# jihun1998/AO

Hardware: AMD Instinct MI355X
Metric: points/sec fwd+bwd PTv2m2 S3DIS (higher is better)
Workload: dtype fp32

## Files before the change

ao_amd/csrc/gva_fwd_tile.hip:

```cpp
#include <algorithm>
#include <cstdlib>

#include "gva_common.h"

namespace gva {

typedef float ft_v4f __attribute__((ext_vector_type(4)));
__device__ __forceinline__ ft_v4f ft_mfma(float a, float b, ft_v4f c) { return __builtin_amdgcn_mfma_f32_16x16x4f32(a, b, c, 0, 0, 0); }
template <int CTRL>
__device__ __forceinline__ float ft_dpp(float v) {
    return __int_as_float(__builtin_amdgcn_update_dpp(0, __float_as_int(v), CTRL, 0xF, 0xF, true));
}
__device__ __forceinline__ float ft_row16_sum(float v) {
    v += ft_dpp<0xB1>(v);
    v += ft_dpp<0x4E>(v);
    v += ft_dpp<0x141>(v);
    v += ft_dpp<0x140>(v);
    return v;
}
__device__ __forceinline__ float ft_row16_max(float v) {
    v = fmaxf(v, ft_dpp<0xB1>(v));
    v = fmaxf(v, ft_dpp<0x4E>(v));
    v = fmaxf(v, ft_dpp<0x141>(v));
    v = fmaxf(v, ft_dpp<0x140>(v));
    return v;
}
__device__ __forceinline__ void ft_wave_sync() {
    asm volatile("s_waitcnt lgkmcnt(0)" ::: "memory");
    __builtin_amdgcn_wave_barrier();
}

__host__ __device__ constexpr int ft_ww_pitch(int G) {
    int p = G;
    while (p % 16 != 4) ++p;
    return p;
}
__host__ __device__ constexpr int ft_point_pitch(int GB, int GP) {
    int p = GB * GP;
    while (p % 64 != 4) p += 4;
    return p;
}

template <int G, int C, int GB>
struct FwdTileCfg {
    static constexpr int GTF = (G + 15) / 16, G16 = GTF * 16, GPW = ft_ww_pitch(G), QB = GB / 4, NGW = GB / 4, OB = 8 * GB,
                         NCH = C / 16, GP = 20, PP = ft_point_pitch(GB, GP), OP = OB + 4, WT = 16 * 17;
    static_assert(GB % 4 == 0 && GB <= 16 && G % GB == 0 && C == 8 * G && GPW >= G16, "group blocks of 4 q groups");
    static constexpr size_t lds_floats = 4 * (size_t)C + 4 * 256 + 16 * GPW + 16 + 2 * G16 + 16 * WT + 256 + 2 * 16 * PP + 16 * OP;
};

template <int G, int C, int GB, bool WRITE_A, bool DROP>
__global__ __launch_bounds__(256, 2) void attention_fwd_tile_kernel(
    int n, const float *__restrict__ W1, const float *__restrict__ sc, const float *__restrict__ sh, const float *__restrict__ Ww2,
    const float *__restrict__ bw2, const float *__restrict__ v, const float *__restrict__ a, const float *__restrict__ b,
    const float *__restrict__ coord, const int *__restrict__ idx, const float *__restrict__ Wp2, const float *__restrict__ bp2,
    float *__restrict__ w, float *__restrict__ sw, float *__restrict__ out, float *__restrict__ stats, float *__restrict__ a_out,
    PtvDrop drop) {
    using K = FwdTileCfg<G, C, GB>;
    constexpr int GTF = K::GTF, G16 = K::G16, GPW = K::GPW, QB = K::QB, NGW = K::NGW, OB = K::OB, NCH = K::NCH, GP = K::GP, PP = K::PP,
                  OP = K::OP, WT = K::WT;
    extern __shared__ float4 lds4[];
    float4 *sAB = lds4;
    float4 *sPos = sAB + C;
    float *sWw = (float *)(sPos + 256);
    float *sBw = sWw + 16 * GPW;
    float *sSc = sBw + 16;
    float *sSh = sSc + G16;
    float *sWt = sSh + G16;
    float *sSw = sWt + 16 * WT;
    float *sA = sSw + 256;
    float *sOut = sA + 2 * 16 * PP;

    const int tid = threadIdx.x, lane = tid & 63, wid = tid >> 6, l15 = lane & 15, q = lane >> 4;
    const int tile = blockIdx.x, g0 = blockIdx.y * GB, o0 = 8 * g0;
    const long long last = (long long)n - 1;

    long long pts[4];
    int srcv[4];
    float u[4][GTF][4];
#pragma unroll
    for (int i = 0; i < 4; ++i) {
        const long long pt = (long long)tile * 16 + 4 * wid + i;
        pts[i] = pt < n ? pt : last;
        srcv[i] = idx[pts[i] * 16 + l15];
        const float *row = W1 + (pts[i] * 16 + l15) * G;
#pragma unroll
        for (int t = 0; t < GTF; ++t) {
            const int j0 = 16 * t + 4 * q;
            const float4 uu = *(const float4 *)(row + (j0 < G ? j0 : 0));
            u[i][t][0] = j0 < G ? uu.x : 0.f; u[i][t][1] = j0 < G ? uu.y : 0.f;
            u[i][t][2] = j0 < G ? uu.z : 0.f; u[i][t][3] = j0 < G ? uu.w : 0.f;
        }
    }
    for (int ch = tid; ch < C; ch += 256) sAB[ch] = make_float4(a[3 * ch], a[3 * ch + 1], a[3 * ch + 2], b[ch]);
    for (int e = tid; e < 16 * GPW; e += 256) {
        const int row = e / GPW, j = e - row * GPW;
        sWw[e] = (row < GB && j < G) ? Ww2[(g0 + row) * G + j] : 0.f;
    }
    if (tid < 16) sBw[tid] = tid < GB ? bw2[g0 + tid] : 0.f;
    for (int j = tid; j < G16; j += 256) { sSc[j] = j < G ? sc[j] : 0.f; sSh[j] = j < G ? sh[j] : 0.f; }
    float cx[4], cy[4], cz[4];
#pragma unroll
    for (int i = 0; i < 4; ++i) {
        const long long ss = srcv[i] >= 0 ? srcv[i] : 0;
        cx[i] = coord[3 * ss] - coord[3 * pts[i]];
        cy[i] = coord[3 * ss + 1] - coord[3 * pts[i] + 1];
        cz[i] = coord[3 * ss + 2] - coord[3 * pts[i] + 2];
    }
    const int of = lane & 31, par = lane >> 5;
    const bool fa = of < OB / 4;
    auto request_rows = [&](int i, float4 (&rows)[8]) {
#pragma unroll
        for (int j = 0; j < 8; ++j) {
            const int s0 = __builtin_amdgcn_readlane(srcv[i], 2 * j), s1 = __builtin_amdgcn_readlane(srcv[i], 2 * j + 1);
            const int src = par ? s1 : s0;
            const float *vp = (fa && src >= 0) ? v + (long long)src * C + o0 + 4 * of : ptv2_zero_pad;
            rows[j] = *(const float4 *)vp;
        }
    };
    auto reduce_rows = [&](int i, const float4 (&rows)[8]) {
        const int p = 4 * wid + i, gl = fa ? of >> 1 : 0;
        float wg[8];
#pragma unroll
        for (int j = 0; j < 8; ++j) wg[j] = sWt[p * WT + gl * 17 + 2 * j + par];
        float4 acc = make_float4(0.f, 0.f, 0.f, 0.f);
#pragma unroll
        for (int j = 0; j < 8; ++j) {
            acc.x = __builtin_fmaf(wg[j], rows[j].x, acc.x); acc.y = __builtin_fmaf(wg[j], rows[j].y, acc.y);
            acc.z = __builtin_fmaf(wg[j], rows[j].z, acc.z); acc.w = __builtin_fmaf(wg[j], rows[j].w, acc.w);
        }
        acc.x += __shfl_xor(acc.x, 32, WAVE); acc.y += __shfl_xor(acc.y, 32, WAVE);
        acc.z += __shfl_xor(acc.z, 32, WAVE); acc.w += __shfl_xor(acc.w, 32, WAVE);
        if (par == 0 && fa) *(float4 *)(sOut + p * OP + 4 * of) = acc;
    };
    float4 vv0[8], vv1[8];
#ifndef FT_SKIP_OUTV
    request_rows(0, vv0);
    request_rows(1, vv1);
#endif
    __syncthreads();

    ft_v4f z[4];
#pragma unroll
    for (int i = 0; i < 4; ++i) z[i] = (ft_v4f){0.f, 0.f, 0.f, 0.f};
#pragma unroll
    for (int t = 0; t < GTF; ++t) {
        const float4 s4 = *(const float4 *)(sSc + 16 * t + 4 * q), h4 = *(const float4 *)(sSh + 16 * t + 4 * q);
        const float4 w4 = *(const float4 *)(sWw + l15 * GPW + 16 * t + 4 * q);
#pragma unroll
        for (int i = 0; i < 4; ++i) z[i] = ft_mfma(w4.x, fmaxf(__builtin_fmaf(s4.x, u[i][t][0], h4.x), 0.f), z[i]);
#pragma unroll
        for (int i = 0; i < 4; ++i) z[i] = ft_mfma(w4.y, fmaxf(__builtin_fmaf(s4.y, u[i][t][1], h4.y), 0.f), z[i]);
#pragma unroll
        for (int i = 0; i < 4; ++i) z[i] = ft_mfma(w4.z, fmaxf(__builtin_fmaf(s4.z, u[i][t][2], h4.z), 0.f), z[i]);
#pragma unroll
        for (int i = 0; i < 4; ++i) z[i] = ft_mfma(w4.w, fmaxf(__builtin_fmaf(s4.w, u[i][t][3], h4.w), 0.f), z[i]);
    }
    const float4 b4 = *(const float4 *)(sBw + 4 * q);
    const float bb[4] = {b4.x, b4.y, b4.z, b4.w};
#pragma unroll
    for (int i = 0; i < 4; ++i) {
        const int p = 4 * wid + i;
        const bool valid = srcv[i] >= 0;
        float wv[4], so[4];
#pragma unroll
        for (int r = 0; r < 4; ++r) {
            const float zz = z[i][r] + bb[r];
            const float mx = ft_row16_max(zz);
            const float e = expf(zz - mx);
            const float den = ft_row16_sum(e);
            wv[r] = (valid && q < QB) ? e / den : 0.f;
            if (DROP) wv[r] *= ptv2_drop_factor(drop, ((unsigned long long)pts[i] * 16 + l15) * G + (g0 + 4 * q + r));
            so[r] = ft_row16_sum(wv[r]);
            sWt[p * WT + (4 * q + r) * 17 + l15] = wv[r];
        }
        if (q < QB) {
            *(float4 *)(w + (pts[i] * 16 + l15) * G + g0 + 4 * q) = make_float4(wv[0], wv[1], wv[2], wv[3]);
            if (l15 == 0) {
                *(float4 *)(sw + pts[i] * G + g0 + 4 * q) = make_float4(so[0], so[1], so[2], so[3]);
                *(float4 *)(sSw + p * 16 + 4 * q) = make_float4(so[0], so[1], so[2], so[3]);
            }
        }
        sPos[p * 16 + l15] = valid ? make_float4(cx[i], cy[i], cz[i], 0.f) : make_float4(0.f, 0.f, 0.f, 0.f);
    }
    ft_wave_sync();

#ifndef FT_SKIP_OUTV
    reduce_rows(0, vv0);
    reduce_rows(1, vv1);
    request_rows(2, vv0);
    request_rows(3, vv1);
#endif

    float wA[4][4];
    float3 pq[4][4];
#pragma unroll
    for (int i = 0; i < 4; ++i)
#pragma unroll
        for (int st = 0; st < 4; ++st) {
            wA[i][st] = sWt[(4 * wid + i) * WT + l15 * 17 + 4 * st + q];
            const float4 t = sPos[(4 * wid + i) * 16 + 4 * st + q];
            pq[i][st] = make_float3(t.x, t.y, t.z);
        }
    const float *wp2row[NGW];
    float4 wpn[NGW];
    ft_v4f acc[NGW];
#pragma unroll
    for (int gi = 0; gi < NGW; ++gi) {
        const int g = wid + 4 * gi;
        wp2row[gi] = Wp2 + (size_t)(o0 + 8 * g + (l15 & 7)) * C + 4 * q;
        wpn[gi] = *(const float4 *)wp2row[gi];
        acc[gi] = (ft_v4f){0.f, 0.f, 0.f, 0.f};
    }
#ifdef FT_SKIP_CHUNKS
    __syncthreads();
#else
#pragma unroll 2
    for (int ck = 0; ck < NCH; ++ck) {
        float *buf = sA + (ck & 1) * 16 * PP;
        float4 wpc[NGW];
        const int cn = ck + 1 < NCH ? ck + 1 : ck;
#pragma unroll
        for (int gi = 0; gi < NGW; ++gi) { wpc[gi] = wpn[gi]; wpn[gi] = *(const float4 *)(wp2row[gi] + 16 * cn); }
        const float4 ab = sAB[16 * ck + l15];
        ft_v4f d[4];
#pragma unroll
        for (int i = 0; i < 4; ++i) d[i] = (ft_v4f){0.f, 0.f, 0.f, 0.f};
#pragma unroll
        for (int st = 0; st < 4; ++st)
#pragma unroll
            for (int i = 0; i < 4; ++i)
                d[i] = ft_mfma(wA[i][st], pe_act(ab.x, ab.y, ab.z, ab.w, pq[i][st].x, pq[i][st].y, pq[i][st].z), d[i]);
        if (q < QB) {
#pragma unroll
            for (int i = 0; i < 4; ++i)
#pragma unroll
                for (int r = 0; r < 4; ++r) buf[(4 * wid + i) * PP + (4 * q + r) * GP + l15] = d[i][r];
            if constexpr (WRITE_A) {
#pragma unroll
                for (int i = 0; i < 4; ++i)
#pragma unroll
                    for (int r = 0; r < 4; ++r) a_out[(pts[i] * G + g0 + 4 * q + r) * C + 16 * ck + l15] = d[i][r];
            }
        }
        __syncthreads();
#pragma unroll
        for (int gi = 0; gi < NGW; ++gi) {
            const float4 bx = *(const float4 *)(buf + l15 * PP + (wid + 4 * gi) * GP + 4 * q);
            acc[gi] = ft_mfma(wpc[gi].x, bx.x, acc[gi]);
            acc[gi] = ft_mfma(wpc[gi].y, bx.y, acc[gi]);
            acc[gi] = ft_mfma(wpc[gi].z, bx.z, acc[gi]);
            acc[gi] = ft_mfma(wpc[gi].w, bx.w, acc[gi]);
        }
    }
#endif

#ifndef FT_SKIP_OUTV
    reduce_rows(2, vv0);
    reduce_rows(3, vv1);
#endif
    __syncthreads();
    const long long ptl = (long long)tile * 16 + l15;
    const bool rv = ptl < n;
    const int cnt = (int)std::min<long long>(16, (long long)n - (long long)tile * 16);
    const float inv = 1.0f / (float)cnt;
#pragma unroll
    for (int gi = 0; gi < NGW; ++gi) {
        const int g = wid + 4 * gi;
        if (q < 2) {
            const int ol = 8 * g + 4 * q;
            const float4 ov = *(const float4 *)(sOut + l15 * OP + ol);
            const float s = sSw[l15 * 16 + g];
            const float4 bb = *(const float4 *)(bp2 + o0 + ol);
            float4 val;
            val.x = ov.x + acc[gi][0] + bb.x * s; val.y = ov.y + acc[gi][1] + bb.y * s;
            val.z = ov.z + acc[gi][2] + bb.z * s; val.w = ov.w + acc[gi][3] + bb.w * s;
            if (rv) *(float4 *)(out + ptl * C + o0 + ol) = val;
            if (stats) {
                const float s0 = ft_row16_sum(rv ? val.x : 0.f), s1 = ft_row16_sum(rv ? val.y : 0.f);
                const float s2 = ft_row16_sum(rv ? val.z : 0.f), s3 = ft_row16_sum(rv ? val.w : 0.f);
                const float d0 = rv ? val.x - s0 * inv : 0.f, d1 = rv ? val.y - s1 * inv : 0.f;
                const float d2 = rv ? val.z - s2 * inv : 0.f, d3 = rv ? val.w - s3 * inv : 0.f;
                const float m0 = ft_row16_sum(d0 * d0), m1 = ft_row16_sum(d1 * d1), m2 = ft_row16_sum(d2 * d2), m3 = ft_row16_sum(d3 * d3);
                if (l15 == 0) {
                    float *rec = stats + (size_t)tile * 2 * C + o0 + ol;
                    *(float4 *)rec = make_float4(s0, s1, s2, s3);
                    *(float4 *)(rec + C) = make_float4(m0, m1, m2, m3);
                }
            }
        }
    }
}

template <int G, int C, int GB>
static int launch_fwd_tile(int n, const float *W1, const float *sc, const float *sh, const float *Ww2, const float *bw2, const float *v,
                           const float *a, const float *b, const float *coord, const int *idx, const float *Wp2, const float *bp2,
                           float *w, float *sw, float *out, float *stats, float *a_out, PtvDrop drop, hipStream_t st) {
    using K = FwdTileCfg<G, C, GB>;
    const size_t lds = sizeof(float) * K::lds_floats;
    const bool dropping = drop.thresh != 0;
    auto kern = a_out ? (dropping ? attention_fwd_tile_kernel<G, C, GB, true, true> : attention_fwd_tile_kernel<G, C, GB, true, false>)
                      : (dropping ? attention_fwd_tile_kernel<G, C, GB, false, true> : attention_fwd_tile_kernel<G, C, GB, false, false>);
    static bool configured[2][2] = {{false, false}, {false, false}};
    if (!configured[a_out != nullptr][dropping]) {
        if (hipFuncSetAttribute((const void *)kern, hipFuncAttributeMaxDynamicSharedMemorySize, (int)lds) != hipSuccess) return PTV2_ERR_LAUNCH;
        configured[a_out != nullptr][dropping] = true;
    }
    hipLaunchKernelGGL(kern, dim3((n + 15) / 16, G / GB), dim3(256), lds, st, n, W1, sc, sh, Ww2, bw2, v, a, b, coord, idx, Wp2, bp2, w,
                       sw, out, stats, a_out, drop);
    return PTV2_OK;
}

}

int gva_fwd_tile_supported(int k, int c, int g) {
    return k == 16 && ((g == 12 && c == 96) || (g == 24 && c == 192) || (g == 48 && c == 384) || (g == 64 && c == 512));
}
int gva_fwd_tile_stat_rows() { return 16; }

int gva_fwd_tile_launch(int n, int k, int c, int g, const float *W1, const float *sc, const float *sh, const float *Ww2,
                        const float *bw2, const float *v, const float *a, const float *b, const float *coord, const int *idx,
                        const float *Wp2, const float *bp2, float *w, float *sw, float *out, float *stats, float *a_out, void *stream) {
    using namespace gva;
    if (!gva_fwd_tile_supported(k, c, g) || n < 1) return PTV2_ERR_ARG;
    hipStream_t st = (hipStream_t)stream;
    PtvScopedTimer t(KID_FWD_TILE + (g == 12 ? 0 : g == 24 ? 1 : g == 48 ? 2 : 3), st,
                     4.0 * ((double)n * k * (2 * g + 1) + (double)n * (3 + 2 * c + g)));
    int rc;
    const PtvDrop drop = ptv2_attn_drop_current();
#define ARGS n, W1, sc, sh, Ww2, bw2, v, a, b, coord, idx, Wp2, bp2, w, sw, out, stats, a_out, drop, st
    if (g == 12) rc = launch_fwd_tile<12, 96, 12>(ARGS);
    else if (g == 24) rc = launch_fwd_tile<24, 192, 12>(ARGS);
    else if (g == 48) rc = launch_fwd_tile<48, 384, 12>(ARGS);
    else rc = launch_fwd_tile<64, 512, 16>(ARGS);
#undef ARGS
    if (rc != PTV2_OK) return rc;
    PTV2_CHECK_LAUNCH();
    return PTV2_OK;
}

extern "C" int gva_attention_forward_hip_launcher(int n, int k, int c, int g, const float *W1, const float *sc, const float *sh,
                                                  const float *Ww2, const float *bw2, const float *v, const float *a,
                                                  const float *b, const float *coord, const int *idx, const float *Wp2,
                                                  const float *bp2, float *w, float *sw, float *out, float *A, void *stream) {
    if (!W1 || !sc || !sh || !Ww2 || !bw2 || !v || !a || !b || !coord || !idx || !Wp2 || !bp2 || !w || !sw || !out) return PTV2_ERR_ARG;
    if (n == 0) return PTV2_OK;
    return gva_fwd_tile_launch(n, k, c, g, W1, sc, sh, Ww2, bw2, v, a, b, coord, idx, Wp2, bp2, w, sw, out, nullptr, A, stream);
}
```

Baseline: 12.81 million.

## Choose forward tile group-block geometry per size to balance CU wave rounds

Turns the forward attention tile kernel into a 1D-grid dispatcher that can run two group-block sizes in one launch. The first tiles use the wide block, the tail uses GB=4. A host-side planner picks the block sizes and split point from the CU count, using a simple cost model (rounds × (fixed + GB)) to cut tail-wave imbalance. An environment override is added. The cost is more template instantiations, a max-LDS allocation across both configs, and divide/mod index math per block.

```diff
diff --git a/ao_amd/csrc/gva_fwd_tile.hip b/ao_amd/csrc/gva_fwd_tile.hip
--- a/ao_amd/csrc/gva_fwd_tile.hip
+++ b/ao_amd/csrc/gva_fwd_tile.hip
@@ -1,5 +1,6 @@
 #include <algorithm>
 #include <cstdlib>
+#include <cstring>
 
 #include "gva_common.h"
 
@@ -50,12 +51,12 @@
 };
 
 template <int G, int C, int GB, bool WRITE_A, bool DROP>
-__global__ __launch_bounds__(256, 2) void attention_fwd_tile_kernel(
+__device__ __forceinline__ void attention_fwd_tile_body(
     int n, const float *__restrict__ W1, const float *__restrict__ sc, const float *__restrict__ sh, const float *__restrict__ Ww2,
     const float *__restrict__ bw2, const float *__restrict__ v, const float *__restrict__ a, const float *__restrict__ b,
     const float *__restrict__ coord, const int *__restrict__ idx, const float *__restrict__ Wp2, const float *__restrict__ bp2,
     float *__restrict__ w, float *__restrict__ sw, float *__restrict__ out, float *__restrict__ stats, float *__restrict__ a_out,
-    PtvDrop drop) {
+    PtvDrop drop, const int tile, const int g0) {
     using K = FwdTileCfg<G, C, GB>;
     constexpr int GTF = K::GTF, G16 = K::G16, GPW = K::GPW, QB = K::QB, NGW = K::NGW, OB = K::OB, NCH = K::NCH, GP = K::GP, PP = K::PP,
                   OP = K::OP, WT = K::WT;
@@ -72,7 +73,7 @@
     float *sOut = sA + 2 * 16 * PP;
 
     const int tid = threadIdx.x, lane = tid & 63, wid = tid >> 6, l15 = lane & 15, q = lane >> 4;
-    const int tile = blockIdx.x, g0 = blockIdx.y * GB, o0 = 8 * g0;
+    const int o0 = 8 * g0;
     const long long last = (long long)n - 1;
 
     long long pts[4];
@@ -292,23 +293,83 @@
     }
 }
 
-template <int G, int C, int GB>
-static int launch_fwd_tile(int n, const float *W1, const float *sc, const float *sh, const float *Ww2, const float *bw2, const float *v,
-                           const float *a, const float *b, const float *coord, const int *idx, const float *Wp2, const float *bp2,
-                           float *w, float *sw, float *out, float *stats, float *a_out, PtvDrop drop, hipStream_t st) {
-    using K = FwdTileCfg<G, C, GB>;
-    const size_t lds = sizeof(float) * K::lds_floats;
+template <int G, int C, int GB1, int GB2, bool WRITE_A, bool DROP>
+__global__ __launch_bounds__(256, 2) void attention_fwd_tile_kernel(
+    int n, int nt1, int nwg1, const float *__restrict__ W1, const float *__restrict__ sc, const float *__restrict__ sh,
+    const float *__restrict__ Ww2, const float *__restrict__ bw2, const float *__restrict__ v, const float *__restrict__ a,
+    const float *__restrict__ b, const float *__restrict__ coord, const int *__restrict__ idx, const float *__restrict__ Wp2,
+    const float *__restrict__ bp2, float *__restrict__ w, float *__restrict__ sw, float *__restrict__ out, float *__restrict__ stats,
+    float *__restrict__ a_out, PtvDrop drop) {
+    const int bid = blockIdx.x;
+    if (GB1 == GB2 || bid < nwg1) {
+        attention_fwd_tile_body<G, C, GB1, WRITE_A, DROP>(n, W1, sc, sh, Ww2, bw2, v, a, b, coord, idx, Wp2, bp2, w, sw, out, stats,
+                                                          a_out, drop, bid % nt1, bid / nt1 * GB1);
+    } else if constexpr (GB1 != GB2) {
+        const int nt2 = (n + 15) / 16 - nt1, r = bid - nwg1;
+        attention_fwd_tile_body<G, C, GB2, WRITE_A, DROP>(n, W1, sc, sh, Ww2, bw2, v, a, b, coord, idx, Wp2, bp2, w, sw, out, stats,
+                                                          a_out, drop, nt1 + r % nt2, r / nt2 * GB2);
+    }
+}
+
+template <int G, int C, int GB1, int GB2>
+static int launch_fwd_tile(int n, int nt1, const float *W1, const float *sc, const float *sh, const float *Ww2, const float *bw2,
+                           const float *v, const float *a, const float *b, const float *coord, const int *idx, const float *Wp2,
+                           const float *bp2, float *w, float *sw, float *out, float *stats, float *a_out, PtvDrop drop, hipStream_t st) {
+    const size_t lds = sizeof(float) * std::max(FwdTileCfg<G, C, GB1>::lds_floats, FwdTileCfg<G, C, GB2>::lds_floats);
     const bool dropping = drop.thresh != 0;
-    auto kern = a_out ? (dropping ? attention_fwd_tile_kernel<G, C, GB, true, true> : attention_fwd_tile_kernel<G, C, GB, true, false>)
-                      : (dropping ? attention_fwd_tile_kernel<G, C, GB, false, true> : attention_fwd_tile_kernel<G, C, GB, false, false>);
+    auto kern = a_out ? (dropping ? attention_fwd_tile_kernel<G, C, GB1, GB2, true, true> : attention_fwd_tile_kernel<G, C, GB1, GB2, true, false>)
+                      : (dropping ? attention_fwd_tile_kernel<G, C, GB1, GB2, false, true> : attention_fwd_tile_kernel<G, C, GB1, GB2, false, false>);
     static bool configured[2][2] = {{false, false}, {false, false}};
     if (!configured[a_out != nullptr][dropping]) {
         if (hipFuncSetAttribute((const void *)kern, hipFuncAttributeMaxDynamicSharedMemorySize, (int)lds) != hipSuccess) return PTV2_ERR_LAUNCH;
         configured[a_out != nullptr][dropping] = true;
     }
-    hipLaunchKernelGGL(kern, dim3((n + 15) / 16, G / GB), dim3(256), lds, st, n, W1, sc, sh, Ww2, bw2, v, a, b, coord, idx, Wp2, bp2, w,
-                       sw, out, stats, a_out, drop);
+    const int nt = (n + 15) / 16;
+    if (GB1 == GB2) nt1 = nt;
+    const int nwg1 = nt1 * (G / GB1), nwg = nwg1 + (nt - nt1) * (G / GB2);
+    hipLaunchKernelGGL(kern, dim3(nwg), dim3(256), lds, st, n, nt1, nwg1, W1, sc, sh, Ww2, bw2, v, a, b, coord, idx, Wp2, bp2, w, sw,
+                       out, stats, a_out, drop);
     return PTV2_OK;
+}
+
+struct FtPlan { int gb1, gb2, nt1; };
+constexpr int FT_FIXED = 16;
+
+static int ft_cus() {
+    static const int cus = [] {
+        int dev = 0, c = 0;
+        if (hipGetDevice(&dev) != hipSuccess || hipDeviceGetAttribute(&c, hipDeviceAttributeMultiprocessorCount, dev) != hipSuccess || c < 1) c = 256;
+        return c;
+    }();
+    return cus;
+}
+static const char *ft_geom_env() {
+    static const char *e = [] { const char *v = getenv("AO_AMD_FT_GEOM"); return (v && v[0] && strcmp(v, "auto") != 0) ? v : (const char *)nullptr; }();
+    return e;
+}
+static FtPlan ft_plan(int n, int G, int gbdef, const int *cands, int ncand) {
+    const int nt = (n + 15) / 16, cus = ft_cus();
+    auto rounds = [cus](long long wg) { return (long long)((wg + cus - 1) / cus); };
+    auto whole = [&](int gb) { return (long long)nt * (G / gb) / cus * cus / (G / gb); };
+    if (const char *e = ft_geom_env()) {
+        const int gb = e[0] == '0' ? gbdef : atoi(e);
+        bool ok = false;
+        for (int i = 0; i < ncand; ++i) ok |= cands[i] == gb;
+        if (!ok) return FtPlan{gbdef, gbdef, nt};
+        if (strchr(e, '+') && gb == cands[0] && gb != 4) return FtPlan{gb, 4, (int)whole(gb)};
+        return FtPlan{gb, gb, nt};
+    }
+    FtPlan best{gbdef, gbdef, nt};
+    long long bestc = -1, bestwg = 0;
+    auto consider = [&](int gb1, int gb2, long long nt1) {
+        const long long wg1 = nt1 * (G / gb1), wg2 = (nt - nt1) * (G / gb2);
+        const long long c = rounds(wg1) * (FT_FIXED + gb1) + rounds(wg2) * (FT_FIXED + gb2);
+        if (bestc < 0 || c < bestc || (c == bestc && wg1 + wg2 < bestwg)) { bestc = c; bestwg = wg1 + wg2; best = FtPlan{gb1, gb2, (int)nt1}; }
+    };
+    for (int i = 0; i < ncand; ++i) consider(cands[i], cands[i], nt);
+    const int gbw = cands[0];
+    for (long long k = 1; k * cus / (G / gbw) < nt; ++k) consider(gbw, 4, k * cus / (G / gbw));
+    return best;
 }
 
 }
@@ -326,13 +387,29 @@
     hipStream_t st = (hipStream_t)stream;
     PtvScopedTimer t(KID_FWD_TILE + (g == 12 ? 0 : g == 24 ? 1 : g == 48 ? 2 : 3), st,
                      4.0 * ((double)n * k * (2 * g + 1) + (double)n * (3 + 2 * c + g)));
-    int rc;
+    int rc = PTV2_ERR_ARG;
     const PtvDrop drop = ptv2_attn_drop_current();
-#define ARGS n, W1, sc, sh, Ww2, bw2, v, a, b, coord, idx, Wp2, bp2, w, sw, out, stats, a_out, drop, st
-    if (g == 12) rc = launch_fwd_tile<12, 96, 12>(ARGS);
-    else if (g == 24) rc = launch_fwd_tile<24, 192, 12>(ARGS);
-    else if (g == 48) rc = launch_fwd_tile<48, 384, 12>(ARGS);
-    else rc = launch_fwd_tile<64, 512, 16>(ARGS);
+#define ARGS n, p.nt1, W1, sc, sh, Ww2, bw2, v, a, b, coord, idx, Wp2, bp2, w, sw, out, stats, a_out, drop, st
+#define PLAN(G_, C_, A_, B_) if (p.gb1 == A_ && p.gb2 == B_) rc = launch_fwd_tile<G_, C_, A_, B_>(ARGS)
+    if (g == 12) {
+        static const int cand[] = {12, 4};
+        const FtPlan p = ft_plan(n, 12, 12, cand, 2);
+        PLAN(12, 96, 12, 12); else PLAN(12, 96, 4, 4); else PLAN(12, 96, 12, 4);
+    } else if (g == 24) {
+        static const int cand[] = {12, 8, 4};
+        const FtPlan p = ft_plan(n, 24, 12, cand, 3);
+        PLAN(24, 192, 12, 12); else PLAN(24, 192, 8, 8); else PLAN(24, 192, 4, 4); else PLAN(24, 192, 12, 4);
+    } else if (g == 48) {
+        static const int cand[] = {16, 12, 8, 4};
+        const FtPlan p = ft_plan(n, 48, 12, cand, 4);
+        PLAN(48, 384, 16, 16); else PLAN(48, 384, 12, 12); else PLAN(48, 384, 8, 8); else PLAN(48, 384, 4, 4);
+        else PLAN(48, 384, 16, 4);
+    } else {
+        static const int cand[] = {16, 8, 4};
+        const FtPlan p = ft_plan(n, 64, 16, cand, 3);
+        PLAN(64, 512, 16, 16); else PLAN(64, 512, 8, 8); else PLAN(64, 512, 4, 4); else PLAN(64, 512, 16, 4);
+    }
+#undef PLAN
 #undef ARGS
     if (rc != PTV2_OK) return rc;
     PTV2_CHECK_LAUNCH();
```

Result: no change. 12.87 million (median of 6 runs) (+0.5%).
